# AlwinEsch/pvr.rtl.radiofm

Hardware: AMD Instinct MI355X
Metric: IQ MS/s demodulated (whole node) + achieved HBM GB/s on FIR stage (higher is better)
Workload: dtype f32

## Files before the change

### pvr.rtl.radiofm_amd/csrc/fmd_batch.hip

```cpp
#include "../../include/fmd.h"

#include <hip/hip_runtime.h>
#include <hip/hip_ext.h>

#include <algorithm>
#include <chrono>
#include <cmath>
#include <cstdio>
#include <cstdlib>
#include <cstring>
#include <functional>
#include <map>
#include <memory>
#include <mutex>
#include <string>
#include <utility>
#include <vector>

#include "fmd_call_plan.hpp"
#include "fmd_design.hpp"
#include "fmd_groups.hpp"
#include "fmd_kernels.hip.h"
#include "fmd_receiver.hpp"

// ... 185 lines not shown
static_assert(IQ_F32 == FMD_IQ_F32 && IQ_U8 == FMD_IQ_U8 && IQ_S8 == FMD_IQ_S8 && IQ_S16 == FMD_IQ_S16,
              "the plan's formats are the C ABI's");

enum FormatKind { FMT_IQ, FMT_PCM, FMT_MPX, FMT_FEED, FMT_CIQ, FMT_KINDS };
constexpr FormatKind kOutKinds[4] = {FMT_PCM, FMT_MPX, FMT_FEED, FMT_CIQ};
struct FormatInfo
{
  int last;
  unsigned char esz[4];
  const char* must;
};
const FormatInfo kFormats[5] = {
    {FMD_IQ_S16, {8, 2, 2, 4}, "iq_format must be one of FMD_IQ_F32, _U8, _S8, _S16 (0..3)"},
    {FMD_PCM_S16, {4, 2}, "pcm_format must be FMD_PCM_F32 or FMD_PCM_S16 (0..1)"},
    {FMD_MPX_S16, {4, 2}, "mpx_format must be FMD_MPX_F32 or FMD_MPX_S16 (0..1)"},
    {FMD_FEED_S16, {4, 2}, "feed_format must be FMD_FEED_F32 or FMD_FEED_S16 (0..1)"},
    {FMD_CIQ_S16, {8, 4}, "ciq.format must be FMD_CIQ_F32 or FMD_CIQ_S16 (0..1)"}};

inline bool format_ok(FormatKind k, int format)
{
  return format >= 0 && format <= kFormats[k].last;
}

inline size_t format_esz(FormatKind k, int format)
{
  return kFormats[k].esz[format];
}

static_assert(FMD_REAL_F32 == (16 | FMD_IQ_F32) && FMD_REAL_S8 == (16 | FMD_IQ_S8) && FMD_REAL_S16 == (16 | FMD_IQ_S16),
              "a real format is its IQ format with bit 4 set");
inline bool real_format_ok(int format)
{
  return format == FMD_REAL_F32 || format == FMD_REAL_S8 || format == FMD_REAL_S16;
}

inline size_t real_format_esz(int format)
{
  return kFormats[FMT_IQ].esz[format & 3] / 2;
}

static_assert(FMD_IN_CIQ_F32 == (32 | FMD_CIQ_F32) && FMD_IN_CIQ_S16 == (32 | FMD_CIQ_S16),
              "a channel-IQ input format is its output format with bit 5 set");
inline bool ciq_in_format(int format)
{
  return format == FMD_IN_CIQ_F32 || format == FMD_IN_CIQ_S16;
}
const char* const kCiqInOnlyCall =
    "FMD_IN_CIQ_F32 / _S16 (channel IQ rows as input) are taken by the _call entry points only "
    "(fmd_batch_process_device_call, fmd_batch_process_host_call, fmd_process_stream_call)";

struct Out
{
  FormatKind kind;
  void* p = nullptr;
  int fmt = 0;
  size_t stride = 0;
  unsigned* out = nullptr;
  bool deliver = true;
  size_t esz() const { return format_esz(kind, fmt); }
  bool rows_aligned() const { return !(reinterpret_cast<uintptr_t>(p) % 16) && !(stride % (16 / esz())); }
  Out from_channel(unsigned ch0, bool selection) const
  {
    Out o = *this;
    if (p && !selection)
      o.p = static_cast<char*>(p) + size_t(ch0) * stride * esz();
    return o;
  }
};

struct Call
{
  const void* iq = nullptr;
  int iq_fmt = FMD_IQ_F32;
  size_t iq_stride = 0;
  unsigned samples = 0;
  bool from_record = false;
  bool ciq_in() const { return ciq_in_format(iq_fmt); }
  size_t in_esz() const { return ciq_in() ? format_esz(FMT_CIQ, iq_fmt & 1) : format_esz(FMT_IQ, iq_fmt); }
  Out audio{FMT_PCM}, mpx{FMT_MPX}, feed{FMT_FEED}, ciq{FMT_CIQ};
  void* stream = nullptr;
  static constexpr Out Call::* kOut[FMT_KINDS] = {nullptr, &Call::audio, &Call::mpx, &Call::feed, &Call::ciq};
  Out& out(FormatKind k) { return this->*kOut[k]; }
  const Out& out(FormatKind k) const { return this->*kOut[k]; }
};

}

struct fmd_batch
{
  fmd::Params params;
  fmd::Design des;
  unsigned C = 0, CP = 0;
  int device = 0;
  fmd_callbacks cb{};
  void* user = nullptr;
  std::vector<int> shifts;

  static constexpr int NSLOT = kSlots;

  unsigned if_pos = 0;
  unsigned lut_idx = 0;
  float rs_pos = 0.0f;
  unsigned rds_lpf_g = 0;
  unsigned mf_g = 0;
  unsigned alpf_g = 0;
  int hist_sel = 0;
  uint32_t call_index = 0;

  unsigned min_samples = 0;
  int streams_sharing = 0;
  unsigned cpc = 1;
  unsigned Mmax = 0, Mstride = 0, Amax = 0, Rmax = 0;
  std::vector<unsigned> hb_nmax;
  unsigned lastM = 0, lastA = 0, lastR = 0;

  DevBuf<float2> lut, hist[2], demod[2], br[2], mix[2], rdsraw[2], rlpf[2], rs[2], alp[2];
  std::vector<DevBuf<float2>> hbbuf;
  DevBuf<float> if_coeff, rs_coeff, rds_lpf_taps, mf_taps2, audio_taps, ktab;
  DevBuf<float> rpll, rmf, tap_sync;
  DevBuf<double> sctab, sctab256;
  DevBuf<int> pidx;
  static constexpr unsigned kBrFront = 32;
  float2* brp(int q) const { return br[q].p + size_t(kBrFront) * CP; }
  unsigned rs_margin = 0, rs_row = 0;
  int rsr_R = 0, rsr_NW = 0;
  unsigned rsr_nbr = 0, rsr_nbm = 0;
  int rsr_rb = 0;
  DevBuf<float> rsr_tab;
  DevBuf<int> rsr_head, rsr_steps;
  int rsr_mode = -1;
  int n_cus = 256;
  struct HbfPlan
  {
    unsigned n_in = 0, S = 0;
    DevBuf<fmd::HbStep> steps;
    DevBuf<int> seg_first;
  };
  std::vector<std::unique_ptr<HbfPlan>> hbf_plans;
  DevBuf<float2> hbf_tail1, hbf_tail2;
  int hbf_mode = -1;
  static constexpr unsigned kOscH = 64;
  DevBuf<fmd::HbOsc> osc_tab[4];
  HostBuf<fmd::HbOsc> h_osc;
  Event osc_ev[NSLOT];
  size_t h_osc_stride = 0;
  float osc_re = 1.0f, osc_im = 0.0f;
  bool osc_on = false;
  int dbg_nomix = 1;
  int dbg_fir_nt = 0;
  int dbg_serial_claim = 0;
  int dbg_hb4 = 1, dbg_ring4 = 1;
  int dbg_fir_ro = 2;
  bool dbg_fir_interior = true;
  int dbg_lpf_late = -1;
  double host_ms[4] = {0, 0, 0, 0};
  unsigned host_calls = 0;
  DevBuf<long long> serial_probe;
  int dbg_stage_mask = 63;
  DevBuf<float> fstate;
  DevBuf<int> istate;
  DevBuf<uint16_t> r_data;
  SlotQueues<fmd::RdsGroupRec, 1> groups;
  uint32_t drained_call[NSLOT] = {};
  int rb_mode = 0;
  DevBuf<unsigned> rb_quality;
  SlotQueues<uint4, 2> blocks;
  bool rb_dirty[NSLOT] = {};
  Event ev_drained[NSLOT];
  bool drained_pending[NSLOT] = {};
  static constexpr unsigned kExportCursors = 16;
  DevBuf<unsigned> export_cursor;
  unsigned export_seq = 0;
  fmd::ChannelState st{};
  std::vector<fmd::HbCoef> hbcoef;
  fmd::HbChainTaps hb_taps{};

  DevBuf<float> h_stage[FMT_KINDS];
  int dbg_mpx_timing = 0;
  Event mpx_ev[NSLOT][2];
  DevBuf<unsigned long long> pcm_clip;

  struct SelTable
  {
    DevBuf<int> d;
    HostBuf<int> h;
    Event read;
    hipStream_t stream = nullptr;
  };
  struct Selection
  {
    bool on = false;
    unsigned n_total = 0;
    std::vector<unsigned> list;
    std::vector<int2> ent;
    bool dirty = false;
    std::vector<std::unique_ptr<SelTable>> pool;
    int cur = -1;
  };
  Selection sel[FMT_KINDS];
  unsigned feed_div = 0, feed_T = 0;
  uint64_t feed_g = 0;
  std::vector<float> feed_taps_h;
  DevBuf<float> feed_taps, feed_x;
  Event feed_done;
  hipStream_t feed_stream = nullptr;
  int dbg_feed_skip_roll = 0;
  int dbg_ciq_in_skip = 0;
  bool decoder_owned = false;

  std::vector<std::unique_ptr<fmd::GroupDecoder>> gdec;

  int profiling = 0;
  int write_taps = 0;

  int concurrency = 1;
  hipStream_t s_fir = nullptr, s_ser = nullptr, s_post = nullptr, s_rds = nullptr, s_lpf = nullptr;
  std::vector<std::unique_ptr<fmd_batch>> subs;
  std::vector<unsigned> sub_ch0;
  bool owns_streams = true;
  hipEvent_t vheavy[2] = {nullptr, nullptr};
  hipEvent_t sched_prev2 = nullptr;
  bool split_post = false;
  bool serial_exclusive = false;
  enum { EV_IN, EV_FIR, EV_INDONE, EV_SER, EV_AUD, EV_RDS, EV_HEAVY, EV_RDSH, EV_ALP, EV_DEC, EV_ROLL, EV_N };
  Event cev[NSLOT][EV_N];
  uint32_t slot_call[NSLOT] = {};
  std::vector<Event> ev;
  unsigned prof_calls = 0;

  HostBuf<unsigned> h_err;
  bool failed = false;
  std::string fail_msg;
  unsigned spin_limit = 1u << 20;
  bool if_dry_run = false;
  HostBuf<unsigned> h_status;
  DevBuf<unsigned> d_status;
  unsigned host_seq = 0;

  fmd_params cparams{};
  std::unique_ptr<fmd_batch> twin;
  DevBuf<float2> twin_iq;
  DevBuf<float> twin_audio;
  std::mutex log_mu;
  std::vector<std::vector<std::pair<uint32_t, int>>> shift_log;
  std::vector<std::vector<uint32_t>> retune_log;
  std::vector<uint32_t> gdec_epoch;
  struct Edit
  {
    unsigned ch;
    int shift;
    bool reset;
    int imp = -1;
  };
  std::vector<Edit> edits;
  bool edits_pending = false;
  fmd::RestartTable restart_tab{};
  int restart_group[fmd::kRestartMaxRegions] = {};
  int restart_skip = -1;
  unsigned restart_rows_cap = 0;
  HostBuf<int2> h_edits;
  HostBuf<float2> h_rows;
  DevBuf<int2> d_edits;
  DevBuf<float2> d_rows;
  Event edit_ev[NSLOT];
  Event edit_done;
  unsigned restart_seq = 0;
  DevBuf<unsigned> org;
  bool origins_live = false;
  int dbg_reset_keep_phase = 0;

  unsigned n_cap = 0;
  bool map_on = false, map_dirty = false;
  int capture_walk = 1;
  std::vector<unsigned> cmap;
  DevBuf<uint2> d_walk;
  HostBuf<uint2> h_walk;
  Event walk_ev[NSLOT];

  fmd::StateTable state_tab{};
  int state_group[fmd::kStateMaxRegions] = {};
  size_t state_bytes = 0;
  int state_skip = -1;
  struct PendingImport
  {
    int slot = 0;
    unsigned n_cols = 0, n_rows = 0;
    size_t rows_at = 0, payload_at = 0, bytes = 0;
    bool origins_live = false;
    std::vector<fmd::StateEdit> list;
  };
  std::vector<PendingImport> imports;
  HostBuf<char> h_imp[NSLOT];
  DevBuf<char> d_imp[NSLOT];
  Event imp_ev[NSLOT];
  unsigned imp_seq = 0;
  struct GdecImport
  {
    uint32_t k = 0;
    std::unique_ptr<fmd::GroupDecoder> g;
  };
  std::map<unsigned, std::vector<GdecImport>> gdec_imports;
  unsigned osc_warm = 0;

  ~fmd_batch()
  {
    (void)hipSetDevice(device);
// ... 1499 lines not shown
  return fmd_batch_process_device_fmt(b, d_iq, FMD_IQ_F32, iq_channel_stride, samples, d_audio, audio_channel_stride,
                                      out_floats, stream);
}

int fmd_batch_process_device_u8(fmd_batch* b, const uint8_t* d_iq_u8, size_t iq_channel_stride,
                                unsigned samples, float* d_audio, size_t audio_channel_stride,
                                unsigned* out_floats, void* stream)
{
  return fmd_batch_process_device_fmt(b, d_iq_u8, FMD_IQ_U8, iq_channel_stride, samples, d_audio,
                                      audio_channel_stride, out_floats, stream);
}

static bool slot_eligible(const fmd_batch* b, int q, int lag)
{
  return b->slot_call[q] != 0 && b->slot_call[q] + uint32_t(lag) <= b->call_index;
}

static int wait_impl(fmd_batch* b, int lag, void* stream_, bool take_lost)
{
  if (!b || lag < 0 || lag > 4)
    return fail(FMD_ERR_ARG, "fmd_batch_wait: bad argument (lag must be 0..4)");
  hipStream_t stream = static_cast<hipStream_t>(stream_);
  HIPCHK(hipSetDevice(b->device));
  if (is_shell(b))
  {
    for (auto& sb : b->subs)
    {
      const int rc = wait_impl(sb.get(), lag, stream_, false);
      if (rc < 0)
        return check_device_errors(b);
    }
    if (int rc = check_device_errors(b))
      return rc;
    return take_lost ? take_lost_groups(b) : FMD_OK;
  }
  auto wait_if_pending = [&](hipEvent_t e) {
    if (hipEventQuery(e) == hipSuccess)
      return hipSuccess;
    (void)hipGetLastError();
    return hipStreamWaitEvent(stream, e, 0);
  };
  for (int q = 0; q < fmd_batch::NSLOT; q++)
    if (slot_eligible(b, q, lag))
    {
      HIPCHK(wait_if_pending(b->cev[q][fmd_batch::EV_AUD]));
      HIPCHK(wait_if_pending(b->cev[q][fmd_batch::EV_RDS]));
      HIPCHK(wait_if_pending(b->cev[q][fmd_batch::EV_INDONE]));
      HIPCHK(wait_if_pending(b->cev[q][fmd_batch::EV_ROLL]));
    }
  if (int rc = check_device_errors(b))
    return rc;
  return take_lost ? take_lost_groups(b) : FMD_OK;
}

int fmd_batch_wait_lagged(fmd_batch* b, int lag, void* stream_)
{
  return wait_impl(b, lag, stream_, true);
}

int fmd_batch_take_rds_lost(fmd_batch* b)
{
  if (!b)
    return fail(FMD_ERR_ARG, "null batch");
  return take_lost_groups(b) == FMD_WARN_RDS_LOST ? 1 : 0;
}

int fmd_batch_debug_set_spin_limit(fmd_batch* b, unsigned limit)
{
  if (!b)
    return fail(FMD_ERR_ARG, "null batch");
  set_all(b, &fmd_batch::spin_limit, limit);
  b->st.spin_limit = limit;
  for (auto& sb : b->subs)
    sb->st.spin_limit = limit;
  return FMD_OK;
}

int fmd_batch_debug_restart_skip(fmd_batch* b, int region)
{
  if (!b)
    return fail(FMD_ERR_ARG, "null batch");
  if (region < -1 || region >= kRestartRegionCount)
  {
    std::string names;
    for (const char* r : kRestartRegions)
      names += std::string(names.empty() ? "" : ", ") + r;
    return fail(FMD_ERR_ARG, "fmd_batch_debug_restart_skip: -1 or the index of a region (" + names + ")");
  }
  set_all(b, &fmd_batch::restart_skip, region);
  return FMD_OK;
}

int fmd_batch_debug_reset_keep_ring_phase(fmd_batch* b, int on)
{
  if (!b)
    return fail(FMD_ERR_ARG, "null batch");
  set_all(b, &fmd_batch::dbg_reset_keep_phase, on != 0);
  return FMD_OK;
}

int fmd_batch_debug_host_ms(fmd_batch* b, float out[4])
{
  if (!b || !out)
    return fail(FMD_ERR_ARG, "null argument");
  const unsigned n = b->host_calls;
  for (int i = 0; i < 4; i++)
  {
    out[i] = n ? float(b->host_ms[i] / n) : 0.0f;
    b->host_ms[i] = 0.0;
  }
  b->host_calls = 0;
  return int(n);
}

int fmd_batch_debug_set(fmd_batch* b, const char* key, int value)
{
  if (!b || !key)
    return fail(FMD_ERR_ARG, "null argument");
  const std::string k(key);
  HIPCHK(hipSetDevice(b->device));
  HIPCHK(hipDeviceSynchronize());
  if (is_shell(b))
  {
    for (auto& sb : b->subs)
      if (int rc = fmd_batch_debug_set(sb.get(), key, value))
        return rc;
    return FMD_OK;
  }
  if (k == "resampler")
  {
    if (value > 0 && b->rsr_R == 0)
      return fail(FMD_ERR_ARG, "fmd_batch_debug_set: no form of k_resample_ring fits this geometry");
    b->rsr_mode = value < 0 ? -1 : (value ? 1 : 0);
  }
  else if (k == "fir_nt")
    b->dbg_fir_nt = std::max(0, value);
  else if (k == "serial_claim")
    b->dbg_serial_claim = value != 0;
  else if (k == "serial_exclusive")
    b->serial_exclusive = value != 0;
  else if (k == "split_post")
    b->split_post = value != 0;
  else if (k == "hb4")
    b->dbg_hb4 = value != 0;
  else if (k == "ring4")
    b->dbg_ring4 = value != 0;
  else if (k == "lpf_late")
    b->dbg_lpf_late = value < 0 ? -1 : std::min(value, 2);
  else if (k == "stage_mask")
    b->dbg_stage_mask = value & 63;
  else if (k == "fir_ro")
  {
    const int ro = value < 0 ? -value : value;
    b->dbg_fir_ro = (ro == 2 || ro == 3) ? ro : 1;
    b->dbg_fir_interior = value >= 0;
  }
  else if (k == "serial_probe")
  {
    HIPCHK(hipSetDevice(b->device));
    HIPCHK(hipDeviceSynchronize());
    b->serial_probe.release();
    if (value && b->serial_probe.alloc(size_t(8) * 3 * (b->CP / 64)))
      return fail(FMD_ERR_DEVICE, "serial probe allocation failed");
  }
  else if (k == "halfband_chain")
  {
    b->hbf_mode = value < 0 ? -1 : (value ? 1 : 0);
    if (value > 0 && b->call_index == 0 && b->h_osc.p && b->des.hb.size() == 3 &&
        b->des.hb[0].len - 1 <= int(fmd_batch::kOscH))
      b->osc_on = true;
  }
  else if (k == "nomix")
    b->dbg_nomix = value != 0;
  else if (k == "rsr_form")
  {
    bool ok = false;
    for (int f = std::max(0, std::min(2, value)); f < 3 && !ok; f++)
      ok = rsr_configure(b, f);
  }
  else
    return fail(FMD_ERR_ARG, "fmd_batch_debug_set: unknown key '" + k + "'");
  return FMD_OK;
}

int fmd_batch_enable_retune(fmd_batch* b)
{
  if (!b)
    return fail(FMD_ERR_ARG, "fmd_batch_enable_retune: null batch");
  if (b->twin)
    return FMD_OK;
  if (b->call_index != 0)
    return fail(FMD_ERR_STATE, "fmd_batch_enable_retune: only before the batch's first call");
  HIPCHK(hipSetDevice(b->device));
  fmd_batch* tw = nullptr;
  const int zero_shift = 0;
  if (int rc = create_one(&b->cparams, 1, &zero_shift, b->device, nullptr, nullptr, b, &tw))
    return rc;
  std::unique_ptr<fmd_batch> twin(tw);
  twin->concurrency = 2;
  if (b->twin_iq.alloc(FMD_MAX_BLOCK) || b->twin_audio.alloc(fmd_batch_max_audio_floats(tw, FMD_MAX_BLOCK)))
    return fail(FMD_ERR_DEVICE, "fmd_batch_enable_retune: device allocation failed");
  for (const Part& p : parts(b))
    if (int rc = build_restart_table(p.x, tw))
      return rc;
  HIPCHK(hipDeviceSynchronize());
  {
    std::lock_guard<std::mutex> lk(b->log_mu);
    b->shift_log.resize(b->C);
  }
  b->gdec_epoch.resize(b->C, 0u);
  b->twin = std::move(twin);
  return FMD_OK;
}

int fmd_batch_retune_channels(fmd_batch* b, const unsigned* channels, const int* shifts, unsigned n)
{
  if (!b || !channels || !shifts)
    return fail(FMD_ERR_ARG, "fmd_batch_retune_channels: null argument");
  if (b->failed)
    return fail(FMD_ERR_ARG, "fmd_batch_retune_channels: the batch has failed (fmd_batch_reset clears it)");
  if (!b->twin)
    return fail(FMD_ERR_STATE, "fmd_batch_retune_channels: retuning is not enabled (fmd_batch_enable_retune)");
  if (int rc = check_channel_list(b, channels, nullptr, n, "fmd_batch_retune_channels"))
    return rc;
  const uint32_t k = b->call_index + 1;
  std::lock_guard<std::mutex> lk(b->log_mu);
  for (unsigned i = 0; i < n; i++)
  {
    unsigned lc = 0;
    fmd_batch* ob = owner_of(b, channels[i], &lc);
    ob->edits.push_back(fmd_batch::Edit{lc, shifts[i], false});
    drop_gdec_import(b, channels[i], k);
    auto& log = b->shift_log[channels[i]];
    if (!log.empty() && log.back().first == k)
      log.back().second = shifts[i];
    else
      log.emplace_back(k, shifts[i]);
    if (b->retune_log.size() < b->C)
      b->retune_log.resize(b->C);
    auto& rlog = b->retune_log[channels[i]];
    if (rlog.empty() || rlog.back() != k)
      rlog.push_back(k);
  }
  b->edits_pending = true;
  return FMD_OK;
}

int fmd_batch_reset_channels(fmd_batch* b, const unsigned* channels, unsigned n)
{
  if (!b || !channels)
    return fail(FMD_ERR_ARG, "fmd_batch_reset_channels: null argument");
  if (b->failed)
    return fail(FMD_ERR_ARG, "fmd_batch_reset_channels: the batch has failed (fmd_batch_reset clears it)");
  std::vector<unsigned> seen(channels, channels + n);
  std::sort(seen.begin(), seen.end());
  if (n && seen.back() >= b->C)
    return fail(FMD_ERR_ARG, "fmd_batch_reset_channels: channel " + std::to_string(seen.back()) + " out of range");
  if (std::adjacent_find(seen.begin(), seen.end()) != seen.end())
    return fail(FMD_ERR_ARG, "fmd_batch_reset_channels: a channel is listed twice");
  if (n == 0)
    return FMD_OK;
  const uint32_t k = b->call_index + 1;
  std::lock_guard<std::mutex> lk(b->log_mu);
  if (b->shift_log.empty())
  {
    b->shift_log.resize(b->C);
    b->gdec_epoch.assign(b->C, 0u);
  }
  for (unsigned i = 0; i < n; i++)
  {
    unsigned lc = 0;
    fmd_batch* ob = owner_of(b, channels[i], &lc);
    ob->edits.push_back(fmd_batch::Edit{lc, 0, true});
    drop_gdec_import(b, channels[i], k);
    auto& log = b->shift_log[channels[i]];
    if (log.empty() || log.back().first != k)
      log.emplace_back(k, log.empty() ? b->shifts[channels[i]] : log.back().second);
  }
  b->edits_pending = true;
  return FMD_OK;
}

int fmd_batch_wait(fmd_batch* b, void* stream_)
{
  return fmd_batch_wait_lagged(b, 0, stream_);
}

int fmd_batch_set_channels_per_capture(fmd_batch* b, unsigned channels_per_capture)
{
  if (!b)
    return fail(FMD_ERR_ARG, "null batch");
  const unsigned k = channels_per_capture ? channels_per_capture : 1u;
  if (b->C % k)
    return fail(FMD_ERR_ARG, "fmd_batch_set_channels_per_capture: the channel count is not a multiple of it");
  for (size_t i = 0; i < b->subs.size(); i++)
    if (b->sub_ch0[i] % k || b->subs[i]->C % k)
      return fail(FMD_ERR_ARG, "fmd_batch_set_channels_per_capture: with " + std::to_string(b->C) +
                                   " channels the batch runs as sub-batches of " + std::to_string(b->subs[0]->C) +
                                   ", which is not a multiple of it");
  HIPCHK(hipSetDevice(b->device));
  HIPCHK(hipDeviceSynchronize());
  set_all(b, &fmd_batch::cpc, k);
  set_all(b, &fmd_batch::map_on, false);
  set_all(b, &fmd_batch::n_cap, 0u);
  return FMD_OK;
}

// ... 1437 lines not shown
```

### pvr.rtl.radiofm_amd/csrc/fmd_batch_if.inc.hpp

```cpp
namespace
{

template <class IN>
using FirFn = void (*)(const typename IN::elem*, size_t, unsigned, const float2*, float2*, const float2*,
                       unsigned, unsigned, const float*, unsigned, unsigned, unsigned, unsigned, float2*,
                       unsigned, unsigned, unsigned, unsigned, const uint2*);

template <class IN, int TILE, int E, bool MAP, bool RB128 = false>
int launch_if_stage_t(fmd_batch* b, const void* d_iq, size_t iq_channel_stride, unsigned N, unsigned pos,
                      unsigned M, int q, hipStream_t sF, const std::function<void(int)>& mark,
                      hipEvent_t ev_start, hipEvent_t ev_stop)
{
  const fmd::Design& d = b->des;
  const unsigned C = b->C, D = d.D, T = d.table_size;
  const unsigned ntiles = (M + TILE - 1) / TILE;
  const size_t region = ((size_t(TILE - 1) * D + d.if_order + 2u * (1u << E) + 2u) >> E) + 2u;
  const bool longasm = TILE == 256 && d.if_order >= 512;
  const size_t lds = (region << E) * sizeof(float2) + (longasm ? 32 * sizeof(float2) : 0);
  if (lds > 160 * 1024)
    return fail(FMD_ERR_ARG, "IF filter window does not fit in LDS");
  const bool pow2 = (T & (T - 1)) == 0 && T <= 2u * TILE && (size_t(TILE) * D) % T == 0;
  const unsigned rounds = unsigned(((size_t(TILE - 1) * D + d.if_order + 2) / 2 + TILE - 1) / TILE);
  FirFn<IN> kfn = &fmd::k_if_fir<IN, TILE, 1, false, E, false, false, false, MAP>;
  if (pow2)
    kfn = rounds <= 2 ? &fmd::k_if_fir<IN, TILE, 2, true, E, false, false, false, MAP>
        : rounds <= 4 ? &fmd::k_if_fir<IN, TILE, 4, true, E, false, false, false, MAP>
        : rounds <= 6 ? &fmd::k_if_fir<IN, TILE, 6, true, E, false, false, false, MAP>
        : rounds <= 7 ? &fmd::k_if_fir<IN, TILE, 7, true, E, false, false, false, MAP>
                      : &fmd::k_if_fir<IN, TILE, 8, true, E, false, false, false, MAP>;
  if (pow2 && longasm)
    kfn = &fmd::k_if_fir<IN, TILE, 8, true, E, TILE == 256 && (E == 0 || RB128), false,
                         TILE == 256 && RB128 && (E >= 1), MAP>;
  const bool shfl = b->params.fir_reduction == 1 && TILE == 64 && E == 0 && pow2 && rounds <= 8;
  if (shfl)
    kfn = &fmd::k_if_fir<IN, TILE, 8, true, E, false, TILE == 64 && E == 0, false, MAP>;
  const bool fma = b->params.fir_reduction == 2;
  const int fir_nt = fma ? 2 : b->dbg_fir_nt ? b->dbg_fir_nt : (b->concurrency == 2 && b->serial_exclusive ? 2 : 1);
  unsigned nblocks = C * ntiles, ntiles_l = ntiles;
  size_t lds_l = lds;
  FirFn<IN> kfn3 = nullptr;
  if (TILE == 64 && E == 0 && pow2 && rounds == 7 && fir_nt > 1 && !shfl)
  {
    const unsigned nt = fir_nt >= 8 ? 8u : fir_nt >= 4 ? 4u : fir_nt == 3 ? 3u : 2u;
    kfn = nt == 8 ? &fmd::k_if_fir_mt<IN, 7, 8, MAP>
        : nt == 4 ? &fmd::k_if_fir_mt<IN, 7, 4, MAP>
        : nt == 3 ? &fmd::k_if_fir_mt<IN, 7, 3, MAP>
                  : &fmd::k_if_fir_mt<IN, 7, 2, MAP>;
    nblocks = C * ((ntiles + nt - 1) / nt);
    const unsigned RO = fma ? 2u : unsigned(b->dbg_fir_ro), T3 = 64 * RO;
    const unsigned rounds3 = unsigned(((size_t(T3 - 1) * D + d.if_order + 2) / 2 + 63) / 64);
    if (RO > 1 && nt == 2 && d.if_order == 88 && D == 11 && (size_t(T3) * D) % T == 0 &&
        rounds3 <= (RO == 3 ? 18u : 12u))
    {
      kfn3 = RO == 3 ? &fmd::k_if_fir_mt3<IN, 18, 2, 3, 88, 11, false, MAP>
             : fma   ? &fmd::k_if_fir_mt3<IN, 12, 2, 2, 88, 11, true, MAP>
                     : &fmd::k_if_fir_mt3<IN, 12, 2, 2, 88, 11, false, MAP>;
      ntiles_l = (M + T3 - 1) / T3;
      lds_l = RO == 2 ? size_t(12) * 64 * 2 * sizeof(float2) : (size_t(T3 - 1) * D + d.if_order + 4) * sizeof(float2);
      static_assert(size_t(12) * 64 * 2 >= size_t(127) * 11 + 88 + 4, "the rounds' pairs hold the window");
      nblocks = C * ((ntiles_l + 1) / 2);
    }
  }
  if (fma && !kfn3)
    return fail(FMD_ERR_ARG, "FMD_FIR_FMA_PARITY_WAIVED: the fused multiply-add form exists for the reference geometry "
                             "only (88-tap IF filter, downsample 11, power-of-two tuner table)");
  if (b->if_dry_run)
    return FMD_OK;
  if (lds > 64 * 1024)
    (void)hipFuncSetAttribute(reinterpret_cast<const void*>(kfn),
                              hipFuncAttributeMaxDynamicSharedMemorySize, 160 * 1024);
  const typename IN::elem* x = static_cast<const typename IN::elem*>(d_iq);
  mark(0);
  launch(kfn3 ? kfn3 : kfn, dim3(nblocks), dim3(TILE), unsigned(lds_l), sF, ev_start, ev_stop, x, iq_channel_stride,
         N, b->hist[b->hist_sel].p, b->hist[b->hist_sel ^ 1].p, b->lut.p, T, b->lut_idx, b->if_coeff.p, d.if_order, D,
         pos, M, b->demod[q].p, b->Mstride, ntiles_l,
         ((C % 8 == 0) ? 1u : 0u) | ((kfn3 && !b->dbg_fir_interior) ? 2u : 0u), b->cpc,
         MAP ? (const uint2*)b->d_walk.p : nullptr);
  mark(1);
  hipLaunchKernelGGL((fmd::k_if_level<IN, MAP>), dim3(C), dim3(64), 0, sF, x, iq_channel_stride, N, b->lut.p, T,
                     b->lut_idx, b->st, b->cpc, MAP ? (const uint2*)b->d_walk.p : nullptr);
  return FMD_OK;
}

template <class IN, int TILE, bool MAP>
int launch_if_stage_e(fmd_batch* b, const void* d_iq, size_t iq_channel_stride, unsigned N, unsigned pos,
                      unsigned M, int q, hipStream_t sF, const std::function<void(int)>& mark,
                      hipEvent_t ev_start, hipEvent_t ev_stop)
{
  const unsigned D = b->des.D;
  if (D % 2 != 0)
    return launch_if_stage_t<IN, TILE, 0, MAP>(b, d_iq, iq_channel_stride, N, pos, M, q, sF, mark, ev_start, ev_stop);
  if (D % 4 != 0)
  {
    const unsigned T = b->des.table_size;
    const bool pow2 = (T & (T - 1)) == 0 && T <= 2u * TILE && (size_t(TILE) * D) % T == 0;
    if (TILE == 256 && b->des.if_order >= 512 && pow2)
      return launch_if_stage_t<IN, TILE, 0, MAP>(b, d_iq, iq_channel_stride, N, pos, M, q, sF, mark, ev_start, ev_stop);
    return launch_if_stage_t<IN, TILE, 1, MAP>(b, d_iq, iq_channel_stride, N, pos, M, q, sF, mark, ev_start, ev_stop);
  }
  {
    const unsigned T = b->des.table_size;
    const bool pow2 = (T & (T - 1)) == 0 && T <= 2u * TILE && (size_t(TILE) * D) % T == 0;
    if (TILE == 256 && b->des.if_order >= 512 && pow2)
    {
      if (D % 8 != 0)
        return launch_if_stage_t<IN, TILE, 1, MAP, true>(b, d_iq, iq_channel_stride, N, pos, M, q, sF, mark, ev_start,
                                                    ev_stop);
      return launch_if_stage_t<IN, TILE, 2, MAP, true>(b, d_iq, iq_channel_stride, N, pos, M, q, sF, mark, ev_start,
                                                  ev_stop);
    }
  }
  return launch_if_stage_t<IN, TILE, 2, MAP>(b, d_iq, iq_channel_stride, N, pos, M, q, sF, mark, ev_start, ev_stop);
}

template <class IN, bool MAP>
int launch_if_stage_m(fmd_batch* b, const void* d_iq, size_t iq_channel_stride, unsigned N, unsigned pos,
                      unsigned M, int q, hipStream_t sF, const std::function<void(int)>& mark,
                      hipEvent_t ev_start, hipEvent_t ev_stop)
{
  const fmd::Design& d = b->des;
  const unsigned T = d.table_size;
  auto fits = [&](unsigned tile) {
    const bool pow2 = (T & (T - 1)) == 0 && T <= 2u * tile && (size_t(tile) * d.D) % T == 0;
    const size_t lds = (size_t(tile - 1) * d.D + d.if_order + 4) * sizeof(float2);
    return pow2 && d.if_order <= 4u * tile * d.D / 8u && lds <= 16 * 1024;
  };
  if (fits(64))
    return launch_if_stage_e<IN, 64, MAP>(b, d_iq, iq_channel_stride, N, pos, M, q, sF, mark, ev_start, ev_stop);
  if (fits(128))
    return launch_if_stage_e<IN, 128, MAP>(b, d_iq, iq_channel_stride, N, pos, M, q, sF, mark, ev_start, ev_stop);
  return launch_if_stage_e<IN, 256, MAP>(b, d_iq, iq_channel_stride, N, pos, M, q, sF, mark, ev_start, ev_stop);
}

template <class IN>
int launch_if_stage(fmd_batch* b, const void* d_iq, size_t iq_channel_stride, unsigned N, unsigned pos,
                    unsigned M, int q, hipStream_t sF, const std::function<void(int)>& mark,
                    hipEvent_t ev_start, hipEvent_t ev_stop)
{
  if (b->map_on)
    return launch_if_stage_m<IN, true>(b, d_iq, iq_channel_stride, N, pos, M, q, sF, mark, ev_start, ev_stop);
  return launch_if_stage_m<IN, false>(b, d_iq, iq_channel_stride, N, pos, M, q, sF, mark, ev_start, ev_stop);
}

}
```

### pvr.rtl.radiofm_amd/csrc/fmd_k_if.hip.h

```cpp
#pragma once

#include "fmd_k_common.hip.h"

namespace fmd
{

__device__ __forceinline__ void fir_long_odd_asm(fmd_f2v& acc2, unsigned& a0, unsigned klo, unsigned khi,
                                                 unsigned& cnt)
{
  asm volatile(
      "s_mov_b32 s72, %3\n\t"
      "s_mov_b32 s73, %4\n\t"
      "s_load_dwordx16 s[40:55], s[72:73], 0x0\n\t"
      "ds_read2_b64 v[64:67], %1 offset0:15 offset1:14\n\t"
      "ds_read2_b64 v[68:71], %1 offset0:13 offset1:12\n\t"
      "ds_read2_b64 v[72:75], %1 offset0:11 offset1:10\n\t"
      "ds_read2_b64 v[76:79], %1 offset0:9 offset1:8\n\t"
      "ds_read2_b64 v[80:83], %1 offset0:7 offset1:6\n\t"
      "ds_read2_b64 v[84:87], %1 offset0:5 offset1:4\n\t"
      "ds_read2_b64 v[88:91], %1 offset0:3 offset1:2\n\t"
      "ds_read2_b64 v[92:95], %1 offset0:1\n\t"
      "v_subrev_u32 %1, 128, %1\n\t"
      "s_add_u32 s72, s72, 64\n\t"
      "s_addc_u32 s73, s73, 0\n\t"
// ... 849 lines not shown
  }
}

template <class IN, int UNROLL, int NT, bool MAP = false>
__global__ __launch_bounds__(64) void k_if_fir_mt(const typename IN::elem* __restrict__ iq,
                                                  size_t chan_stride, unsigned N,
                                                  const float2* __restrict__ hist_in,
                                                  float2* __restrict__ hist_out,
                                                  const float2* __restrict__ lut, unsigned T,
                                                  unsigned lut_idx0, const float* __restrict__ coeff,
                                                  unsigned order, unsigned D, unsigned pos, unsigned M,
                                                  float2* __restrict__ out, unsigned Mstride,
                                                  unsigned ntiles, unsigned xcd_map, unsigned cpc,
                                                 const uint2* __restrict__ walk)
{
  typedef typename IN::pair pair_t;
  constexpr int TILE = 64;
  extern __shared__ __attribute__((aligned(16))) float2 win[];
  __builtin_amdgcn_s_setprio(1);
  const unsigned ngroups = (ntiles + NT - 1) / NT;
  unsigned c, tg;
  if (xcd_map)
  {
    const unsigned xcd = blockIdx.x & 7u, slot = blockIdx.x >> 3;
    c = (slot / ngroups) * 8u + xcd;
    tg = slot % ngroups;
  }
  else
  {
    c = blockIdx.x / ngroups;
    tg = blockIdx.x % ngroups;
  }
  const unsigned tid = threadIdx.x;
  unsigned cap;
  if constexpr (MAP)
    cap = walk_take(walk, c);
  else
    cap = capture_of(c, cpc);
  const typename IN::elem* __restrict__ x = iq + (size_t)cap * chan_stride;
  const float2* __restrict__ l = lut + (size_t)c * T;
  const unsigned mask = T - 1;
  const int kfull_all = (int)(N & ~1u);
  float2 l0, l1;
  {
    const int k_al0 = ((int)(pos + tg * NT * TILE * D) - (int)order) & ~1;
    const unsigned li = (lut_idx0 + (unsigned)k_al0 + 2u * tid) & mask;
    l0 = l[li];
    l1 = l[(li + 1) & mask];
  }
  pair_t v[UNROLL];
  auto issue = [&](unsigned tile) {
    const unsigned m0 = tile * TILE;
    const unsigned nout = min((unsigned)TILE, M - m0);
    const int p_first = (int)(pos + m0 * D);
    const int k_lo = p_first - (int)order;
    const int k_hi = p_first + (int)((nout - 1) * D);
    const int k_al = k_lo & ~1;
    const int kfull = min(k_hi, kfull_all);
    const int ifirst = k_al < 0 ? (-k_al) >> 1 : 0;
    const int npairs = (kfull - k_al + 1) >> 1;
    const pair_t* __restrict__ src = reinterpret_cast<const pair_t*>(x) + (k_al >> 1);
#pragma unroll
    for (int u = 0; u < UNROLL; u++)
      v[u] = src[max(min(u * TILE + (int)tid, npairs - 1), ifirst)];
  };
  const unsigned t_first = tg * NT;
  issue(t_first);
  for (unsigned i = 0; i < (unsigned)NT; i++)
  {
    const unsigned tile = t_first + i;
    if (tile >= ntiles)
      break;
    const unsigned m0 = tile * TILE;
    const unsigned nout = min((unsigned)TILE, M - m0);
    const int p_first = (int)(pos + m0 * D);
    const int k_lo = p_first - (int)order;
    const int k_hi = p_first + (int)((nout - 1) * D);
    const int k_al = k_lo & ~1;
    if (k_lo < 0)
    {
      const float2* __restrict__ h = hist_in + (size_t)c * order;
      const int nh = min(-k_lo, k_hi - k_lo);
      for (int q = (int)tid; q < nh; q += TILE)
        win[q + (k_lo - k_al)] = h[(int)order + k_lo + q];
    }
    {
      const int kfull = min(k_hi, kfull_all);
      const int ifirst = k_al < 0 ? (-k_al) >> 1 : 0;
      const int npairs = (kfull - k_al + 1) >> 1;
      float4* dst = reinterpret_cast<float4*>(win);
#pragma unroll
      for (int u = 0; u < UNROLL; u++)
      {
        const int q = u * TILE + (int)tid;
        if (q >= ifirst && q < npairs)
        {
          float2 a, b;
          IN::unpack(v[u], a, b);
          a = cmul(a, l0);
          b = cmul(b, l1);
          dst[q] = make_float4(a.x, a.y, b.x, b.y);
        }
      }
      const pair_t* __restrict__ src = reinterpret_cast<const pair_t*>(x) + (k_al >> 1);
      for (int q = UNROLL * TILE + (int)tid; q < npairs; q += TILE)
      {
        float2 a, b;
        IN::unpack(src[max(q, ifirst)], a, b);
        a = cmul(a, l0);
        b = cmul(b, l1);
        if (q >= ifirst)
          dst[q] = make_float4(a.x, a.y, b.x, b.y);
      }
      for (int k = max(kfull, 0) + (int)tid; k < k_hi; k += TILE)
        win[k - k_al] = cmul(IN::one(x, k), l[(lut_idx0 + (unsigned)k) & mask]);
    }
    lds_wave_sync();
    if (i + 1 < (unsigned)NT && tile + 1 < ntiles)
      issue(tile + 1);
    if (tid < nout)
    {
      float2 acc = make_float2(0.0f, 0.0f);
      const float2* w = win + (k_lo - k_al) + tid * D + order;
#pragma unroll 8
      for (unsigned j = 1; j <= order; j++)
      {
        const float k = coeff[j];
        const float2 sm = w[-(int)j];
        acc.x += sm.x * k;
        acc.y += sm.y * k;
      }
      out[(size_t)c * Mstride + m0 + tid] = acc;
    }
    if (tile == ntiles - 1)
    {
      float2* __restrict__ ho = hist_out + (size_t)c * order;
      const float2* __restrict__ hi = hist_in + (size_t)c * order;
      const unsigned keep = N < order ? order - N : 0u;
      for (unsigned q = tid; q < order; q += TILE)
      {
        if (q < keep)
          ho[q] = hi[q + N];
        else
        {
          const unsigned k = N + q - order;
          ho[q] = cmul(IN::one(x, k), l[(lut_idx0 + k) % T]);
        }
      }
    }
    lds_wave_sync();
  }
}

template <class IN, int UNROLL, int NT, int RO = 3, int ORD = 88, int DEC = 11, bool FMA = false, bool MAP = false>
__global__ __launch_bounds__(64) __attribute__((amdgpu_waves_per_eu(RO == 2 ? 4 : 3)))
void k_if_fir_mt3(const typename IN::elem* __restrict__ iq,
                                                   size_t chan_stride, unsigned N,
                                                   const float2* __restrict__ hist_in,
                                                   float2* __restrict__ hist_out,
                                                   const float2* __restrict__ lut, unsigned T,
                                                   unsigned lut_idx0, const float* __restrict__ coeff,
                                                   unsigned order, unsigned D, unsigned pos, unsigned M,
                                                   float2* __restrict__ out, unsigned Mstride,
                                                   unsigned ntiles, unsigned xcd_map, unsigned cpc,
                                                 const uint2* __restrict__ walk)
{
  typedef typename IN::pair pair_t;
  static_assert(RO == 2 || RO == 3, "outputs per lane (lane stride RO D samples: conflict-free for 3)");
  constexpr int LANES = 64, TILE = LANES * RO;
  extern __shared__ __attribute__((aligned(16))) float2 win[];
  __builtin_amdgcn_s_setprio(1);
  const unsigned ngroups = (ntiles + NT - 1) / NT;
  unsigned c, tg;
  if (xcd_map & 1u)
  {
    const unsigned xcd = blockIdx.x & 7u, slot = blockIdx.x >> 3;
    c = (slot / ngroups) * 8u + xcd;
    tg = slot % ngroups;
  }
  else
  {
    c = blockIdx.x / ngroups;
    tg = blockIdx.x % ngroups;
  }
  const unsigned tid = threadIdx.x;
  unsigned cap;
  if constexpr (MAP)
    cap = walk_take(walk, c);
  else
    cap = capture_of(c, cpc);
  const typename IN::elem* __restrict__ x = iq + uniform_u64((size_t)cap * chan_stride);
  const float2* __restrict__ l = lut + (size_t)c * T;
  const unsigned mask = T - 1;
  const int kfull_all = (int)(N & ~1u);
  float2 l0, l1;
  {
    const int k_al0 = ((int)(pos + tg * NT * TILE * D) - (int)order) & ~1;
    const unsigned li = (lut_idx0 + (unsigned)k_al0 + 2u * tid) & mask;
    l0 = l[li];
    l1 = l[(li + 1) & mask];
  }
  pair_t v[UNROLL];
  auto issue = [&](unsigned tile) {
    const unsigned m0 = tile * TILE;
    const unsigned nout = min((unsigned)TILE, M - m0);
    const int p_first = (int)(pos + m0 * D);
    const int k_lo = p_first - (int)order;
    const int k_hi = p_first + (int)((nout - 1) * D);
    const int k_al = k_lo & ~1;
    const int kfull = min(k_hi, kfull_all);
    const int ifirst = k_al < 0 ? (-k_al) >> 1 : 0;
    const int npairs = (kfull - k_al + 1) >> 1;
    const pair_t* __restrict__ src = reinterpret_cast<const pair_t*>(x) + (k_al >> 1);
#pragma unroll
    for (int u = 0; u < UNROLL; u++)
      v[u] = src[max(min(u * LANES + (int)tid, npairs - 1), ifirst)];
  };
  constexpr bool HAS_INTERIOR = RO == 2;
  constexpr int LDSP = RO == 2 ? UNROLL * LANES : ((TILE - 1) * DEC + ORD + 4) / 2;
  static_assert((LDSP + LANES - 1) / LANES == UNROLL, "the rounds stage one window");
  auto interior = [&](unsigned tile) {
    const unsigned m0 = tile * TILE;
    const int k_lo = (int)(pos + m0 * D) - (int)order;
    return HAS_INTERIOR && !(xcd_map & 2u) && m0 + TILE <= M && k_lo >= 0 && (k_lo & ~1) + 2 * UNROLL * LANES <= kfull_all;
  };
  auto issue_interior = [&](unsigned tile) {
    const int k_al = ((int)(pos + tile * TILE * D) - (int)order) & ~1;
    const pair_t* __restrict__ src = reinterpret_cast<const pair_t*>(x) + (k_al >> 1);
#pragma unroll
    for (int u = 0; u < UNROLL; u++)
      v[u] = src[u * LANES + (int)tid];
  };
  auto run_tile = [&](unsigned tile, auto interior_c, auto next_c, auto first_c) {
    constexpr bool INTERIOR = decltype(interior_c)::value;
    constexpr int NEXT = decltype(next_c)::value;
    if (decltype(first_c)::value)
    {
      if (INTERIOR)
        issue_interior(tile);
      else
        issue(tile);
    }
    const unsigned m0 = tile * TILE;
    const unsigned nout = min((unsigned)TILE, M - m0);
    const int p_first = (int)(pos + m0 * D);
    const int k_lo = p_first - (int)order;
    const int k_hi = p_first + (int)((nout - 1) * D);
    const int k_al = k_lo & ~1;
    if (INTERIOR)
    {
      float4* dst = reinterpret_cast<float4*>(win);
#pragma unroll
      for (int u = 0; u < UNROLL; u++)
      {
        const int q = u * LANES + (int)tid;
        if ((u + 1) * LANES <= LDSP || q < LDSP)
        {
          float2 a, b;
          IN::unpack(v[u], a, b);
          a = cmul_pk(a, l0);
          b = cmul_pk(b, l1);
          dst[q] = make_float4(a.x, a.y, b.x, b.y);
        }
      }
    }
    else
    {
      if (k_lo < 0)
      {
        const float2* __restrict__ h = hist_in + (size_t)c * order;
        const int nh = min(-k_lo, k_hi - k_lo);
        for (int q = (int)tid; q < nh; q += LANES)
          win[q + (k_lo - k_al)] = h[(int)order + k_lo + q];
      }
      const int kfull = min(k_hi, kfull_all);
      const int ifirst = k_al < 0 ? (-k_al) >> 1 : 0;
      const int npairs = (kfull - k_al + 1) >> 1;
      float4* dst = reinterpret_cast<float4*>(win);
#pragma unroll
      for (int u = 0; u < UNROLL; u++)
      {
        const int q = u * LANES + (int)tid;
        if (q >= ifirst && q < npairs)
        {
          float2 a, b;
          IN::unpack(v[u], a, b);
          a = cmul(a, l0);
          b = cmul(b, l1);
          dst[q] = make_float4(a.x, a.y, b.x, b.y);
        }
      }
      const pair_t* __restrict__ src = reinterpret_cast<const pair_t*>(x) + (k_al >> 1);
      for (int q = UNROLL * LANES + (int)tid; q < npairs; q += LANES)
      {
        float2 a, b;
        IN::unpack(src[max(q, ifirst)], a, b);
        a = cmul(a, l0);
        b = cmul(b, l1);
        if (q >= ifirst)
          dst[q] = make_float4(a.x, a.y, b.x, b.y);
      }
      for (int k = max(kfull, 0) + (int)tid; k < k_hi; k += LANES)
        win[k - k_al] = cmul(IN::one(x, k), l[(lut_idx0 + (unsigned)k) & mask]);
    }
    lds_wave_sync();
    if (NEXT == 2)
      issue_interior(tile + 1);
    else if (NEXT == 1)
      issue(tile + 1);
    if (tid * RO < nout)
    {
      static_assert(ORD % DEC == 0 && ORD >= RO * DEC, "stretches of DEC samples");
      constexpr int NB = ORD / DEC, NS = NB + (RO - 1);
      float2 acc[RO];
#pragma unroll
      for (int r = 0; r < RO; r++)
        acc[r] = make_float2(0.0f, 0.0f);
      const float2* w = win + (k_lo - k_al) + (tid * RO + (RO - 1)) * DEC + ORD;
      auto stretch = [&](int st, auto all) {
        const float2* ws = w - st * DEC;
#pragma unroll
        for (int i = 1; i <= DEC; i++)
        {
          const float2 sm = ws[-i];
#pragma unroll
          for (int r = 0; r < RO; r++)
          {
            const int sb = st - (RO - 1 - r);
            if (decltype(all)::value || (sb >= 0 && sb < NB))
            {
              const float cj = coeff[sb * DEC + i];
              if (FMA)
              {
                const fmd_f2v t = __builtin_elementwise_fma(fmd_f2v{sm.x, sm.y}, fmd_f2v{cj, cj},
                                                            fmd_f2v{acc[r].x, acc[r].y});
                acc[r] = make_float2(t.x, t.y);
              }
              else
              {
                acc[r].x += sm.x * cj;
                acc[r].y += sm.y * cj;
              }
            }
          }
        }
      };
#pragma unroll
// ... 103 lines not shown
```

Measured before the change: 297,600.

## Add cross-lane DPP hop path for the 88-tap IF FIR with 121-output tiles

```diff
diff --git a/pvr.rtl.radiofm_amd/csrc/fmd_batch.hip b/pvr.rtl.radiofm_amd/csrc/fmd_batch.hip
--- a/pvr.rtl.radiofm_amd/csrc/fmd_batch.hip
+++ b/pvr.rtl.radiofm_amd/csrc/fmd_batch.hip
@@ -361,6 +361,7 @@
   int dbg_hb4 = 1, dbg_ring4 = 1;
   int dbg_fir_ro = 2;
   bool dbg_fir_interior = true;
+  bool dbg_fir_hop = true;
   int dbg_lpf_late = -1;
   double host_ms[4] = {0, 0, 0, 0};
   unsigned host_calls = 0;
@@ -2166,7 +2167,8 @@
   else if (k == "fir_ro")
   {
     const int ro = value < 0 ? -value : value;
-    b->dbg_fir_ro = (ro == 2 || ro == 3) ? ro : 1;
+    b->dbg_fir_hop = ro == 22;
+    b->dbg_fir_ro = (ro == 2 || ro == 3) ? ro : b->dbg_fir_hop ? 2 : 1;
     b->dbg_fir_interior = value >= 0;
   }
   else if (k == "serial_probe")
diff --git a/pvr.rtl.radiofm_amd/csrc/fmd_batch_if.inc.hpp b/pvr.rtl.radiofm_amd/csrc/fmd_batch_if.inc.hpp
--- a/pvr.rtl.radiofm_amd/csrc/fmd_batch_if.inc.hpp
+++ b/pvr.rtl.radiofm_amd/csrc/fmd_batch_if.inc.hpp
@@ -39,6 +39,7 @@
   unsigned nblocks = C * ntiles, ntiles_l = ntiles;
   size_t lds_l = lds;
   FirFn<IN> kfn3 = nullptr;
+  bool hop = false;
   if (TILE == 64 && E == 0 && pow2 && rounds == 7 && fir_nt > 1 && !shfl)
   {
     const unsigned nt = fir_nt >= 8 ? 8u : fir_nt >= 4 ? 4u : fir_nt == 3 ? 3u : 2u;
@@ -59,6 +60,7 @@
       lds_l = RO == 2 ? size_t(12) * 64 * 2 * sizeof(float2) : (size_t(T3 - 1) * D + d.if_order + 4) * sizeof(float2);
       static_assert(size_t(12) * 64 * 2 >= size_t(127) * 11 + 88 + 4, "the rounds' pairs hold the window");
       nblocks = C * ((ntiles_l + 1) / 2);
+      hop = RO == 2 && !fma && b->dbg_fir_hop;
     }
   }
   if (fma && !kfn3)
@@ -74,7 +76,8 @@
   launch(kfn3 ? kfn3 : kfn, dim3(nblocks), dim3(TILE), unsigned(lds_l), sF, ev_start, ev_stop, x, iq_channel_stride,
          N, b->hist[b->hist_sel].p, b->hist[b->hist_sel ^ 1].p, b->lut.p, T, b->lut_idx, b->if_coeff.p, d.if_order, D,
          pos, M, b->demod[q].p, b->Mstride, ntiles_l,
-         ((C % 8 == 0) ? 1u : 0u) | ((kfn3 && !b->dbg_fir_interior) ? 2u : 0u), b->cpc,
+         ((C % 8 == 0) ? 1u : 0u) | ((kfn3 && !b->dbg_fir_interior) ? 2u : 0u) | (hop ? 4u : 0u),
+         b->cpc,
          MAP ? (const uint2*)b->d_walk.p : nullptr);
   mark(1);
   hipLaunchKernelGGL((fmd::k_if_level<IN, MAP>), dim3(C), dim3(64), 0, sF, x, iq_channel_stride, N, b->lut.p, T,
diff --git a/pvr.rtl.radiofm_amd/csrc/fmd_k_if.hip.h b/pvr.rtl.radiofm_amd/csrc/fmd_k_if.hip.h
--- a/pvr.rtl.radiofm_amd/csrc/fmd_k_if.hip.h
+++ b/pvr.rtl.radiofm_amd/csrc/fmd_k_if.hip.h
@@ -1025,6 +1025,13 @@
   }
 }
 
+__device__ __forceinline__ fmd_f2v hop_down(fmd_f2v a)
+{
+  const int x = __float_as_int(a.x), y = __float_as_int(a.y);
+  return fmd_f2v{__int_as_float(__builtin_amdgcn_update_dpp(x, x, 0x130, 0xf, 0xf, false)),
+                 __int_as_float(__builtin_amdgcn_update_dpp(y, y, 0x130, 0xf, 0xf, false))};
+}
+
 template <class IN, int UNROLL, int NT, int RO = 3, int ORD = 88, int DEC = 11, bool FMA = false, bool MAP = false>
 __global__ __launch_bounds__(64) __attribute__((amdgpu_waves_per_eu(RO == 2 ? 4 : 3)))
 void k_if_fir_mt3(const typename IN::elem* __restrict__ iq,
@@ -1066,6 +1073,166 @@
   const float2* __restrict__ l = lut + (size_t)c * T;
   const unsigned mask = T - 1;
   const int kfull_all = (int)(N & ~1u);
+  if constexpr (RO == 2 && !FMA && ORD == 88 && DEC == 11 && UNROLL == 12)
+  {
+    if (xcd_map & 4u)
+    {
+      constexpr int HT = 121, HS = 22, HW = LANES * HS;
+      constexpr int HR = HW / (2 * LANES);
+      static_assert(HW == (HT - 1) * DEC + ORD && HR * 2 * LANES == HW && HR < UNROLL && HW % 128 == 0, "the window");
+      const unsigned htiles = (M + HT - 1) / HT;
+      const unsigned t_end = tg + 1 == ngroups ? htiles : tg * 2u + 2u;
+      auto k_lo_of = [&](unsigned tile) { return (int)(pos + tile * HT * D) - ORD; };
+      auto hop_interior = [&](unsigned tile) {
+        const int k_lo = k_lo_of(tile);
+        return !(xcd_map & 2u) && tile * HT + HT <= M && k_lo >= 0 && (k_lo & ~1) + HW + 2 <= kfull_all;
+      };
+      pair_t v[HR];
+      typename IN::elem vx;
+      auto hop_issue = [&](unsigned tile) {
+        const int k_al = k_lo_of(tile) & ~1;
+        const pair_t* __restrict__ src = reinterpret_cast<const pair_t*>(x) + (k_al >> 1);
+#pragma unroll
+        for (int u = 0; u < HR; u++)
+          v[u] = src[u * LANES + (int)tid];
+        vx = x[k_al + HW];
+      };
+      if (hop_interior(tg * 2u))
+        hop_issue(tg * 2u);
+#pragma unroll 1
+      for (unsigned tile = tg * 2u; tile < t_end; tile++)
+      {
+        const unsigned m0 = tile * HT;
+        const unsigned nout = min((unsigned)HT, M - m0);
+        const int k_lo = k_lo_of(tile);
+        if (hop_interior(tile))
+        {
+          const int k_al = k_lo & ~1;
+          const unsigned li = (lut_idx0 + (unsigned)k_al + 2u * tid) & mask;
+          const float2 l0 = l[li], l1 = l[(li + 1) & mask];
+          if (k_lo & 1)
+          {
+            float2* const wb = win + 1 + 2 * tid;
+#pragma unroll
+            for (int u = 0; u < HR; u++)
+            {
+              float2 a, b;
+              IN::unpack(v[u], a, b);
+              wb[u * 2 * LANES] = cmul_pk(a, l0);
+              wb[u * 2 * LANES + 1] = cmul_pk(b, l1);
+            }
+            if (tid == 0)
+              win[HW + 1] = cmul_pk(IN::one(&vx, 0), l0);
+          }
+          else
+          {
+            float4* const wb = reinterpret_cast<float4*>(win + 2) + tid;
+#pragma unroll
+            for (int u = 0; u < HR; u++)
+            {
+              float2 a, b;
+              IN::unpack(v[u], a, b);
+              a = cmul_pk(a, l0);
+              b = cmul_pk(b, l1);
+              wb[u * LANES] = make_float4(a.x, a.y, b.x, b.y);
+            }
+          }
+        }
+        else
+        {
+          const float2* __restrict__ h = hist_in + (size_t)c * order;
+          const int k0 = k_lo + (int)tid;
+          const unsigned li = (lut_idx0 + (unsigned)k0) & mask;
+          const float2 la = l[li], lb = l[(li + LANES) & mask];
+          auto part = [&](auto i0_c) {
+            constexpr int I0 = decltype(i0_c)::value;
+            typename IN::elem e[HS / 2];
+#pragma unroll
+            for (int i = 0; i < HS / 2; i++)
+              e[i] = x[min(max(k0 + (I0 + i) * LANES, 0), (int)N - 1)];
+#pragma unroll
+            for (int i = 0; i < HS / 2; i++)
+            {
+              const int k = k0 + (I0 + i) * LANES;
+              float2 sm = cmul(IN::one(&e[i], 0), ((I0 + i) & 1) ? lb : la);
+              if (k >= (int)N)
+                sm = make_float2(0.0f, 0.0f);
+              if ((I0 + i) * LANES < ORD && k < 0)
+                sm = h[ORD + k];
+              win[2 + (int)tid + (I0 + i) * LANES] = sm;
+            }
+          };
+          part(std::integral_constant<int, 0>{});
+          part(std::integral_constant<int, HS / 2>{});
+        }
+        lds_wave_sync();
+        float4 r[HS / 2];
+        {
+          const float4* wl = reinterpret_cast<const float4*>(win + 2) + tid * (HS / 2);
+#pragma unroll
+          for (int i = 0; i < HS / 2; i++)
+            r[i] = wl[i];
+        }
+        if (tile + 1 < t_end && hop_interior(tile + 1))
+          hop_issue(tile + 1);
+        auto taps = [&](fmd_f2v& acc, auto j0_c, auto i0_c, auto n_c) {
+          constexpr int J0 = decltype(j0_c)::value, I0 = decltype(i0_c)::value, NTAP = decltype(n_c)::value;
+#pragma unroll
+          for (int n = 0; n < NTAP; n++)
+          {
+            const int i = I0 - n;
+            const float cj = coeff[J0 + n];
+            const fmd_f2v sm = (i & 1) ? fmd_f2v{r[i >> 1].z, r[i >> 1].w} : fmd_f2v{r[i >> 1].x, r[i >> 1].y};
+            const fmd_f2v pr = sm * fmd_f2v{cj, cj};
+            acc = acc + pr;
+          }
+        };
+        typedef std::integral_constant<int, HS> CS;
+        typedef std::integral_constant<int, HS / 2> CH;
+        typedef std::integral_constant<int, HS - 1> ITOP;
+        typedef std::integral_constant<int, HS / 2 - 1> IMID;
+        fmd_f2v ev = {0.0f, 0.0f}, od = {0.0f, 0.0f};
+        taps(od, std::integral_constant<int, 1>{}, IMID{}, CH{});
+        od = hop_down(od);
+        taps(ev, std::integral_constant<int, 1>{}, ITOP{}, CS{});
+        ev = hop_down(ev);
+        taps(od, std::integral_constant<int, 12>{}, ITOP{}, CS{});
+        od = hop_down(od);
+        taps(ev, std::integral_constant<int, 23>{}, ITOP{}, CS{});
+        ev = hop_down(ev);
+        taps(od, std::integral_constant<int, 34>{}, ITOP{}, CS{});
+        od = hop_down(od);
+        taps(ev, std::integral_constant<int, 45>{}, ITOP{}, CS{});
+        ev = hop_down(ev);
+        taps(od, std::integral_constant<int, 56>{}, ITOP{}, CS{});
+        od = hop_down(od);
+        taps(ev, std::integral_constant<int, 67>{}, ITOP{}, CS{});
+        taps(od, std::integral_constant<int, 78>{}, ITOP{}, CH{});
+        float2* __restrict__ op = out + (size_t)c * Mstride + m0 + tid * 2u;
+        if (tid * 2u < nout)
+          op[0] = make_float2(ev.x, ev.y);
+        if (tid * 2u + 1u < nout)
+          op[1] = make_float2(od.x, od.y);
+      }
+      if (tg + 1 == ngroups)
+      {
+        float2* __restrict__ ho = hist_out + (size_t)c * order;
+        const float2* __restrict__ hi = hist_in + (size_t)c * order;
+        const unsigned keep = N < order ? order - N : 0u;
+        for (unsigned q = tid; q < order; q += LANES)
+        {
+          if (q < keep)
+            ho[q] = hi[q + N];
+          else
+          {
+            const unsigned k = N + q - order;
+            ho[q] = cmul(IN::one(x, k), l[(lut_idx0 + k) % T]);
+          }
+        }
+      }
+      return;
+    }
+  }
   float2 l0, l1;
   {
     const int k_al0 = ((int)(pos + tg * NT * TILE * D) - (int)order) & ~1;
```

Result: no change. 299,000, median of 6 (+0.5%).
